# Wenri/taichi_3d_gaussian_splatting

Measured on AMD Instinct MI355X. Metric: fps fwd+bwd @1920x1080 (run as 1920x1088), 5e5 Gaussians, higher is better.
Workload: dtype f32; 1 GPU; cfg3_headline: synth(N=500000, 1920x1088, sigma0=0.02, sh_deg=3, seed 0), fwd+bwd, 1 view(s) per GPU per step, the 8 poses of BASELINE config 4 cycled (rank r, step k: pose (r + k) mod 8); points=500000, parallelism=view-parallel x1, 1 view(s) per rank per step, all-reduce per step, views_per_rank=1, poses_cycled=8, forward_sizing=predicted, rehearsal=False, backward_hook=True

## Files before the change

taichi_3d_gaussian_splatting_amd/csrc/gs_api.hip:

```cpp
#include "../../include/gs_rasterizer.h"
#include "gs_common.h"

#include <algorithm>
#include <atomic>
#include <chrono>
#include <initializer_list>
#include <mutex>
#include <string>
#include <vector>
#include <cstdio>
#include <cstring>
#include <cstdlib>

static thread_local std::string g_last_error;

static int fail(int code, const std::string& msg)
{
    g_last_error = msg;
    return code;
}

#define HIP_TRY(expr)                                                                              \
    do {                                                                                           \
        hipError_t e__ = (expr);                                                                   \
// ... 55 lines not shown
    double total_ms[KID_COUNT_] = {};
    int64_t launches[KID_COUNT_] = {};
};

int gs_prof_begin(GsProf* p, int kid, hipStream_t s)
{
    if (!p || !((p->mask >> kid) & 1ull)) return -1;
    GsProf::Rec r; r.kid = kid;
    hipEvent_t* ev[2] = { &r.a, &r.b };
    for (hipEvent_t* e : ev) {
        if (!p->spare.empty()) { *e = p->spare.back(); p->spare.pop_back(); }
        else if (hipEventCreate(e) != hipSuccess) return -1;
    }
    (void)hipEventRecord(r.a, s);
    p->recs.push_back(r);
    return (int)p->recs.size() - 1;
}

void gs_prof_end(GsProf* p, int rec, hipStream_t s)
{
    if (!p || rec < 0) return;
    (void)hipEventRecord(p->recs[rec].b, s);
}

#define GS_COUNTER_SLOTS 64
struct gs_ctx {
    int device = 0;
    GsProf prof;
    std::mutex mu;
    int64_t device_bytes = 0;
    std::vector<Frame*> frames;
    int transient = -1;
    DevBuf block_counts, block_offsets, tile_block_sums, hist, scan_tmp, counters, partial, visited, zero_row, sums, loss_ws;
    DevBuf pose_scratch;
    uint8_t visit_gen = 0;
    GsCounters* host_counters = nullptr;
    GsCounters* host_counters_dev = nullptr;
    uint64_t slots_busy = 1ull;
    int32_t ticket = 0;
    int64_t counter_wait_ns = 0;
    struct { bool valid = false; int H = 0, W = 0; uint32_t K = 0; int max_code = 0; } seen;
    DevBuf order_hint;
    int order_hint_T = 0;
    bool has_stream = false;
    hipStream_t last_stream = nullptr;
    hipEvent_t switch_event = nullptr;
};

extern "C" int gs_abi_version(void) { return GS_ABI_VERSION; }
extern "C" const char* gs_last_error(void) { return g_last_error.c_str(); }

extern "C" const char* gs_kernel_names(void)
{
    return "k_filter,k_scan_tiles_publish,k_project,k_keygen,k_sort_hist,"
           "k_sort_rowscan,k_sort_scatter,k_blend_fwd,k_blend_bwd_tile,k_bwd_points,k_sum_rows,k_tile_order,k_blend_bwd_repair";
}

extern "C" int gs_create(int32_t device, gs_ctx** out)
{
    if (!out) return fail(GS_ERR_INVALID_ARGUMENT, "gs_create: out is NULL");
    int count = 0;
    HIP_TRY(hipGetDeviceCount(&count));
    if (device < 0 || device >= count) return fail(GS_ERR_INVALID_ARGUMENT, "gs_create: no such HIP device");
    HIP_TRY(hipSetDevice(device));
    gs_ctx* c = new gs_ctx();
    c->device = device;
    hipError_t e = hipHostMalloc(reinterpret_cast<void**>(&c->host_counters), sizeof(GsCounters) * GS_COUNTER_SLOTS, hipHostMallocMapped | hipHostMallocCoherent);
    if (e != hipSuccess) { delete c; return fail(GS_ERR_HIP, std::string("hipHostMalloc: ") + hipGetErrorString(e)); }
    std::memset(c->host_counters, 0, sizeof(GsCounters) * GS_COUNTER_SLOTS);
    e = hipHostGetDevicePointer(reinterpret_cast<void**>(&c->host_counters_dev), c->host_counters, 0);
    if (e != hipSuccess) { (void)hipHostFree(c->host_counters); delete c; return fail(GS_ERR_HIP, std::string("hipHostGetDevicePointer: ") + hipGetErrorString(e)); }
    e = c->counters.ensure(sizeof(GsCounters), &c->device_bytes);
    if (e == hipSuccess) e = hipMemset(c->counters.p, 0, sizeof(GsCounters));
    if (e == hipSuccess) e = hipEventCreateWithFlags(&c->switch_event, hipEventDisableTiming);
    if (e != hipSuccess) { c->counters.release(&c->device_bytes); (void)hipHostFree(c->host_counters); delete c; return fail(GS_ERR_OUT_OF_MEMORY, "gs_create: counters"); }
    *out = c;
    return GS_OK;
}

extern "C" int gs_destroy(gs_ctx* c)
{
    if (!c) return GS_OK;
    (void)hipSetDevice(c->device);
    (void)hipDeviceSynchronize();
    for (Frame* f : c->frames) { f->bufs.release(&c->device_bytes); delete f; }
    DevBuf* all[] = { &c->block_counts, &c->block_offsets, &c->tile_block_sums, &c->hist, &c->scan_tmp,
                      &c->counters, &c->partial, &c->visited, &c->zero_row, &c->sums, &c->loss_ws, &c->order_hint, &c->pose_scratch };
    for (DevBuf* b : all) b->release(&c->device_bytes);
    for (GsProf::Rec& r : c->prof.recs) { (void)hipEventDestroy(r.a); (void)hipEventDestroy(r.b); }
    for (hipEvent_t e : c->prof.spare) (void)hipEventDestroy(e);
    if (c->switch_event) (void)hipEventDestroy(c->switch_event);
    if (c->host_counters) (void)hipHostFree(c->host_counters);
    delete c;
    return GS_OK;
}

extern "C" int gs_profile_enable(gs_ctx* c, uint64_t kernel_mask)
{
    if (!c) return fail(GS_ERR_INVALID_ARGUMENT, "gs_profile_enable: ctx is NULL");
    std::lock_guard<std::mutex> lock(c->mu);
    c->prof.mask = kernel_mask;
    return GS_OK;
}

extern "C" int gs_profile_read(gs_ctx* c, double* total_ms, int64_t* launches, int32_t n, int32_t reset)
{
    if (!c || !total_ms || !launches) return fail(GS_ERR_INVALID_ARGUMENT, "gs_profile_read: NULL argument");
    std::lock_guard<std::mutex> lock(c->mu);
    HIP_TRY(hipSetDevice(c->device));
    GsProf& p = c->prof;
    for (GsProf::Rec& r : p.recs) {
        HIP_TRY(hipEventSynchronize(r.b));
        float ms = 0.0f;
        HIP_TRY(hipEventElapsedTime(&ms, r.a, r.b));
        p.total_ms[r.kid] += ms; p.launches[r.kid] += 1;
        p.spare.push_back(r.a); p.spare.push_back(r.b);
    }
    p.recs.clear();
    for (int i = 0; i < n && i < KID_COUNT_; ++i) { total_ms[i] = p.total_ms[i]; launches[i] = p.launches[i]; }
    if (reset) for (int i = 0; i < KID_COUNT_; ++i) { p.total_ms[i] = 0.0; p.launches[i] = 0; }
// ... 247 lines not shown
        GsCounters hc;
        if ((rc = read_counters(c, s, pa.ticket, 0, &hc)) != GS_OK) return rc;
        *M_out = hc.M; *K_out = hc.K;
    }
    return GS_OK;
}

static int run_records_stage(gs_ctx* c, Frame* f, const float* records, int64_t m, const gs_config* cfg, hipStream_t s,
                             GsProjectArgs* pa_out)
{
    FrameBufs& B = f->bufs;
    const int T = f->info.n_tiles;
    const size_t Mp = (size_t)(m > 0 ? m : 1);
    const size_t nb = (size_t)((m + 255) / 256);
    const int rc = grow(c, { NEED(B.rec, 64 * Mp), NEED(B.box, 8 * Mp), NEED(B.ntiles, 4 * Mp), NEED(B.depth_codes, 4 * Mp), NEED(B.offsets, 4 * Mp),
                             NEED(B.tile_start, 4 * GS_TILE_INTS(T)), NEED(B.tile_order, 4 * GS_ORDER_INTS(T)),
                             NEED(c->tile_block_sums, 4 * (nb + 1)) });
    if (rc != GS_OK) return rc;
    if (m > 0) HIP_TRY(hipMemcpyAsync(B.rec.p, records, (size_t)m * 64, hipMemcpyDeviceToDevice, s));
    GsProjectArgs pa{};
    pa.prof = &c->prof; pa.N = m; pa.H = f->info.camera_height; pa.W = f->info.camera_width; pa.depth_scale = cfg->depth_to_sort_key_scale;
    pa.v = frame_view(*f);
    pa.tile_block_sums = c->tile_block_sums.as<uint32_t>();
    pa.counters = c->counters.as<GsCounters>();
    pa.host_mirror = c->host_counters_dev; pa.ticket = ++c->ticket;
    if (c->ticket == 0x7fffffff) c->ticket = 0;
    gs_launch_boxes_from_records(pa, (int)m, s, false);
    f->max_tiles_known = false;
    HIP_TRY(hipGetLastError());
    *pa_out = pa;
    return GS_OK;
}

static int run_raster_stage(gs_ctx* c, Frame* f, const GsProjectArgs& pa, int64_t n_rows, int M_bound, uint32_t K_bound, int depth_bits,
                            const gs_config* cfg, const gs_forward_out* out, hipStream_t s, bool publish)
{
    FrameBufs& B = f->bufs;
    const int T = f->info.n_tiles, H = f->info.camera_height, W = f->info.camera_width, tiles_x = (W + GS_TILE - 1) / GS_TILE;
    static const int seg_env = []{ const char* e = getenv("GS_BWD_SEGMENTS"); return e ? (e[0] == '0' ? 0 : 1) : -1; }();
    const bool want_cuts = seg_env >= 0 ? seg_env == 1 : (int64_t)T * waves_per_tile(T) < 6144;
    int cut_cap = 0;
    if (want_cuts && f->info.kept_for_backward && !cfg->rgb_only && K_bound > 0) {
        cut_cap = (int)std::min<uint64_t>((uint64_t)K_bound / GS_SEG + (uint64_t)T + 2, 0x7fffffffu);
        if (const int rc = grow(c, { NEED(B.cuts, (size_t)cut_cap * 256 * sizeof(float4)), NEED(B.cut_mag, (size_t)cut_cap * 256 * sizeof(float2)) }))
            return rc;
    }
    f->cut_cap = cut_cap;
    const int tile_bits = bits_for((uint32_t)(T > 1 ? T - 1 : 1));
    const int key64 = depth_bits + tile_bits > 32 ? 1 : 0;
    if (depth_bits + tile_bits > 63) return fail(GS_ERR_INVALID_ARGUMENT, "sort key needs more than 63 bits");
    const size_t Kp = K_bound > 0 ? K_bound : 1;
    const size_t key_bytes = key64 ? 8 : 4;
    const size_t hist_elems = gs_sort_hist_elems(K_bound);
    if (const int rc = grow(c, { NEED(B.keys_a, key_bytes * Kp), NEED(B.keys_b, key_bytes * Kp), NEED(B.vals_a, 4 * Kp), NEED(B.vals_b, 4 * Kp),
                                 NEED(c->hist, 4 * hist_elems), NEED(c->scan_tmp, 4 * gs_scan_tmp_elems(hist_elems)) }))
        return rc;

    GsBinArgs ba{};
    ba.prof = &c->prof;
    ba.N = n_rows; ba.M = M_bound; ba.K = K_bound; ba.counters = c->counters.as<GsCounters>();
    ba.tiles_x = tiles_x; ba.depth_scale = cfg->depth_to_sort_key_scale;
    ba.depth_bits = depth_bits; ba.key_bits = depth_bits + tile_bits;
    ba.v = frame_view(*f);
    ba.tile_block_sums = pa.tile_block_sums;
    ba.counters_rw = pa.counters; ba.host_mirror = publish ? pa.host_mirror : nullptr; ba.ticket = pa.ticket;
    ba.block_offsets = pa.block_offsets; ba.block_counts = pa.block_counts;
    ba.keys_a = B.keys_a.p; ba.keys_b = B.keys_b.p; ba.key64 = key64;
    ba.vals_a = B.vals_a.as<int32_t>(); ba.vals_b = B.vals_b.as<int32_t>();
    ba.hist = c->hist.as<uint32_t>(); ba.scan_tmp = c->scan_tmp.as<uint32_t>();
    ba.keys_sorted = &f->keys_sorted; ba.vals_sorted = &f->vals_sorted;
    gs_launch_binning(ba, s);
    HIP_TRY(hipGetLastError());

    GsBlendFwdArgs fa{};
    fa.prof = &c->prof;
    fa.H = H; fa.W = W; fa.tiles_x = tiles_x; fa.rgb_only = cfg->rgb_only;
    fa.v = frame_view(*f);
    fa.key64 = key64; fa.depth_bits = depth_bits; fa.K = K_bound; fa.counters = ba.counters;
    fa.image = out->rasterized_image; fa.depth = out->rasterized_depth; fa.acc_alpha = out->pixel_accumulated_alpha;
    fa.last = out->pixel_offset_of_last_effective_point; fa.count = out->pixel_valid_point_count;
    fa.cut_cap = cut_cap;
    static const bool use_hint = []{ const char* e = getenv("GS_FWD_ORDER_HINT"); return !(e && e[0] == '0'); }();
    fa.order_hint = (use_hint && c->order_hint_T == T && T > 0) ? c->order_hint.as<int32_t>() : nullptr;
    gs_launch_blend_fwd(fa, s);
    HIP_TRY(hipGetLastError());
    f->depth_bits = depth_bits;
    f->key64 = key64;
    f->info.sort_key_bits = depth_bits + tile_bits;
    return GS_OK;
}

static int run_forward_tail(gs_ctx* c, Frame* f, const GsProjectArgs& pa, int64_t n_rows, int M_known, const gs_config* cfg,
                            const gs_forward_out* out, hipStream_t s, int* M_out, uint32_t* K_out)
{
    static const bool predict = []{ const char* e = getenv("GS_PREDICT_SIZES"); return !(e && e[0] == '0'); }();
    const int T = f->info.n_tiles, H = f->info.camera_height, W = f->info.camera_width;
    int rc;
    f->info.sizing = GS_SIZING_EXACT;
    *M_out = 0; *K_out = 0u;
    if (n_rows == 0)
        return run_raster_stage(c, f, pa, 0, 0, 0u, 1, cfg, out, s, false);
    const int tile_bits = bits_for((uint32_t)(T > 1 ? T - 1 : 1));
    bool predicted = false;
// ... 156 lines not shown
}

extern "C" int64_t gs_frame_export_count(gs_ctx* c, const gs_frame* h, gs_export what)
{
    if (!c) return -1;
    std::lock_guard<std::mutex> lock(c->mu);
    Frame* f = resolve(c, h);
    if (f && resolve_pending(c, f) != GS_OK) return -1;
    return f ? export_count(f, what) : -1;
}

extern "C" int gs_frame_export(gs_ctx* c, const gs_frame* h, gs_export what, void* dst, gs_stream stream_)
{
    if (!c) return fail(GS_ERR_INVALID_ARGUMENT, "gs_frame_export: ctx is NULL");
    if (!dst) return fail(GS_ERR_INVALID_ARGUMENT, "gs_frame_export: dst is NULL");
    if (what < 0 || what >= GS_X_COUNT_) return fail(GS_ERR_INVALID_ARGUMENT, "gs_frame_export: unknown export id");
    std::lock_guard<std::mutex> lock(c->mu);
    Frame* f;
    int rc;
    if ((rc = lookup(c, h, "gs_frame_export", true, &f)) != GS_OK) return rc;
    if (export_count(f, what) < 0) return fail(GS_ERR_STATE, "gs_frame_export: this frame does not hold that stage");
    hipStream_t s;
    if ((rc = enter_call(c, stream_, &s)) != GS_OK) return rc;
    const GsFrameView v = frame_view(*f);
    if (what == GS_X_RECORDS) {
        if (f->info.n_points_in_camera > 0)
            HIP_TRY(hipMemcpyAsync(dst, v.PA, (size_t)f->info.n_points_in_camera * 64, hipMemcpyDeviceToDevice, s));
        return GS_OK;
    }
    GsExportArgs a{};
    a.what = (int)what; a.N = f->info.n_points; a.M = (int)f->info.n_points_in_camera; a.K = (uint32_t)f->info.n_keys;
    a.T = v.T; a.depth_bits = f->depth_bits; a.key64 = f->key64;
    a.ids = v.ids; a.PA = v.PA; a.PB = v.PB; a.PC = v.PC; a.PD = v.PD;
    a.ntiles = v.ntiles; a.offsets = v.offsets;
    a.keys_sorted = v.keys_sorted; a.vals_sorted = v.vals_sorted;
    a.tile_start = v.tile_start; a.tile_end = v.tile_end; a.mask = v.mask;
    a.dst = dst;
    gs_launch_export(a, s);
    HIP_TRY(hipGetLastError());
    return GS_OK;
}

static int waves_per_tile(int n_tiles)
{
    int G = 1;
    if (const char* e = getenv("GS_BWD_WAVES_PER_TILE")) G = atoi(e);
    else if (n_tiles < 2000) G = 4;
    else if (n_tiles < 6144) G = 2;
    if (G != 1 && G != 2 && G != 4) G = 1;
    return G;
}

static int prepare_backward_blend(gs_ctx* c, const Frame* f, const float* grad_image, const float* acc_alpha, const int32_t* last,
                                  float* mag_image, float4* sums_out, int strict, hipStream_t stream, GsBackwardArgs* a_out)
{
    const uint32_t K = (uint32_t)f->info.n_keys;
    const int G = waves_per_tile(f->info.n_tiles);
    const size_t rows = (size_t)(K > 0 ? K : 1) * (size_t)G;
    const size_t flag_bytes = (rows + 15) / 16 * 16;
    hipError_t e = c->partial.ensure(rows * 12 * sizeof(float), &c->device_bytes);
    if (e != hipSuccess) return fail(GS_ERR_OUT_OF_MEMORY, "backward: partial-sum buffer");
    const size_t Mp = (size_t)(f->info.n_points_in_camera > 0 ? f->info.n_points_in_camera : 1);
    const size_t cap_before = c->visited.cap;
    e = c->visited.ensure(flag_bytes + Mp + 16, &c->device_bytes);
    if (e != hipSuccess) return fail(GS_ERR_OUT_OF_MEMORY, "backward: visited buffer");
    if (c->visited.cap != cap_before || c->visit_gen == 255) {
        HIP_TRY(hipMemsetAsync(c->visited.p, 0, c->visited.cap, stream));
// ... 418 lines not shown
```

taichi_3d_gaussian_splatting_amd/csrc/gs_common.h:

```cpp
#pragma once
#include <hip/hip_runtime.h>
#include <stdint.h>

#define GS_TILE_SZ 16

#define gs_ballot(pred) __builtin_amdgcn_ballot_w64(pred)

#ifdef GS_STATS
extern __device__ unsigned long long gs_stats_counters[32];
extern __device__ unsigned long long gs_stats_wave_times[2 * 65536];
#endif
#if defined(GS_STATS) && GS_STATS >= 2
#define GS_STAT(i, n) do { const unsigned long long gs_stat_n = (unsigned long long)(n); if (threadIdx.x % 64 == 0) atomicAdd(&gs_stats_counters[i], gs_stat_n); } while (0)
#else
#define GS_STAT(i, n) do { } while (0)
#endif
#define GS_REC(ptr, i) (ptr)[(size_t)(i) * 4]
#define GS_BOUNDARY_TILES 3
#define GS_ALPHA_EPS 0.00392156862745098f
#define GS_ALPHA_MAX 0.99f
#define GS_T_STOP 0.0001f
#define GS_NFEAT 56
#ifndef GS_SEG
#define GS_SEG 512
// ... 238 lines not shown
    int tile_ints;
    int32_t* tile_order;
    int32_t* n_heavy;
    const void* keys_sorted; const int32_t* vals_sorted;
    float4* cuts; float2* cut_mag;
};

struct GsProjectArgs {
    GsProf* prof;
    const float* point_cloud; float* features; const int8_t* invalid; const int32_t* object_id;
    int64_t N; const float* q_pc; const float* t_pc; int n_objects; const float* Kmat;
    int H, W; float near_plane, far_plane, depth_scale;
    GsFrameView v;
    int32_t* block_counts; int32_t* block_offsets; uint32_t* tile_block_sums;
    GsCounters* counters;
    GsCounters* host_mirror; int32_t ticket;
};
void gs_launch_project(const GsProjectArgs& a, hipStream_t s, bool publish);
void gs_launch_publish(const GsProjectArgs& a, int n_blocks, hipStream_t s);
void gs_launch_boxes_from_records(const GsProjectArgs& a, int M, hipStream_t s, bool publish);

struct GsBinArgs {
    GsProf* prof;
    int64_t N; int M; uint32_t K; const GsCounters* counters; int tiles_x; float depth_scale; int depth_bits; int key_bits;
    GsFrameView v;
    const uint32_t* tile_block_sums;
    GsCounters* counters_rw; GsCounters* host_mirror; int32_t ticket;
    const int32_t *block_offsets, *block_counts;
    void *keys_a, *keys_b; int32_t *vals_a, *vals_b;
    int key64;
    uint32_t* hist;
    uint32_t* scan_tmp;
    void** keys_sorted; int32_t** vals_sorted;
};
void gs_launch_binning(const GsBinArgs& a, hipStream_t s);
size_t gs_sort_hist_elems(uint32_t K);
size_t gs_scan_tmp_elems(size_t n);

struct GsBlendFwdArgs {
    GsProf* prof;
    int H, W, tiles_x; int rgb_only;
    GsFrameView v;
    int key64, depth_bits; uint32_t K; const GsCounters* counters;
    float* image; float* depth; float* acc_alpha; int32_t* last; int32_t* count;
    int cut_cap;
    const int32_t* order_hint;
};
void gs_launch_blend_fwd(const GsBlendFwdArgs& a, hipStream_t s);

struct GsBackwardArgs {
    GsProf* prof;
    int64_t N; int M; uint32_t K; int H, W, tiles_x;
    GsFrameView v;
    int32_t* order_hint;
    const float* grad_image; const float* acc_alpha; const int32_t* last;
    const float* grad_depth; const float* depth; const float* grad_alpha; int aux;
    int G;
    int item_cap;
    int heavy_factor_x2;
    int strict;
    float* partial;
    uint8_t* visited;
    uint8_t gen;
    uint8_t* touched;
    const float4* zero_row;
    const int32_t* max_tiles_hint;
    float4* sums;
    const float* point_cloud; const float* features; const int32_t* object_id; const float* Kmat;
    int sh_band; float f_color, f_high, f_s, f_q, f_alpha;
    float* grad_pc; float* grad_feat; float* grad_uv; float* mag; float* mag_image; int32_t* n_affected;
    float* hook_gpc; float* hook_gfeat; float* hook_guv; float* hook_mag;
    int32_t* hook_ids; int32_t* hook_ntiles; float* hook_depth; float* hook_uv;
    int32_t* c_num_in_camera; int32_t* c_num_pixels; float* c_vs_grad; float* c_vs_grad_avg; float* c_pos_grad; float* c_pos_grad_norm;
};
void gs_launch_backward_blend(const GsBackwardArgs& a, hipStream_t s);
void gs_launch_backward_points(const GsBackwardArgs& a, hipStream_t s);
size_t gs_pose_scratch_size(int M, int n_objects);
void gs_launch_pose_grad(const GsBackwardArgs& a, int n_objects, void* scratch, float* grad_q, float* grad_t, hipStream_t s);

struct GsExportArgs { int what; int64_t N; int M; uint32_t K; int T; int depth_bits; int key64;
    const int32_t* ids; const float4 *PA, *PB, *PC, *PD; const int32_t* ntiles; const uint32_t* offsets;
    const void* keys_sorted; const int32_t* vals_sorted; const int32_t *tile_start, *tile_end; const int8_t* mask; void* dst; };
void gs_launch_export(const GsExportArgs& a, hipStream_t s);

struct GsLossImage { const float* p; long long sc, sy, sx; int clamp; };
size_t gs_loss_maps_size(int H, int W);
size_t gs_loss_partials_floats(int H, int W);
void gs_launch_loss_forward(const GsLossImage& X, const GsLossImage& Y, int H, int W, float lambda, float* maps, float* partials, float* terms,
                            hipStream_t s);
void gs_launch_loss_backward(const GsLossImage& X, const GsLossImage& Y, int H, int W, float lambda, const float* maps, const float* upstream,
                             const GsLossImage& G, hipStream_t s);
void gs_launch_adam(float* param, const float* grad, float* m, float* v, int64_t n, float lr, float beta1, float beta2, float eps,
                    int64_t step, hipStream_t s);
void gs_launch_reg_value(const float* feat, const int8_t* invalid, int64_t N, float* workspace, float* out, hipStream_t s);
void gs_launch_reg_grad(const float* feat, const int8_t* invalid, int64_t N, const float* value_and_count, const float* upstream,
                        float* grad, hipStream_t s);

__device__ __forceinline__ void gs_controller_add(int64_t n, int32_t npix, float mag, float g0, float g1, float g2,
                                                  int32_t* num_in_camera, int32_t* num_pixels, float* vs_grad, float* vs_grad_avg,
                                                  float* pos_grad, float* pos_grad_norm)
{
    num_in_camera[n] += 1;
    num_pixels[n] += npix;
    vs_grad[n] += mag;
    const float avg = mag / (float)npix;
    vs_grad_avg[n] += (avg != avg) ? 0.0f : avg;
    pos_grad[3 * n] += g0; pos_grad[3 * n + 1] += g1; pos_grad[3 * n + 2] += g2;
    pos_grad_norm[n] += sqrtf(g0 * g0 + g1 * g1 + g2 * g2);
}

#include "../../include/gs_rasterizer.h"
void gs_launch_density_select(const gs_scene& scene, const gs_controller_accumulators& acc, const int32_t* ids, const int32_t* npix,
                              const float* depth, const float* mag, int64_t M, int remove_floaters, const gs_density_config& cfg,
                              const gs_density_plan& plan, hipStream_t s);
// ... 6 lines not shown
```

taichi_3d_gaussian_splatting_amd/csrc/k_binning.hip:

```cpp
#include "gs_common.h"
#include <type_traits>

#ifndef SORT_ROUNDS
#define SORT_ROUNDS 16
#endif
#define SORT_TILE (256 * SORT_ROUNDS)

template <typename KeyT>
__global__ __launch_bounds__(256) void k_keygen(const int32_t* __restrict__ depth_codes, const ushort4* __restrict__ boxes,
                                                const int32_t* __restrict__ ntiles,
                                                const uint32_t* __restrict__ tile_block_sums,
                                                const int32_t* __restrict__ block_offsets, const int32_t* __restrict__ block_counts,
                                                int M, int tiles_x,
                                                float depth_scale, int depth_bits, uint32_t K_cap,
                                                uint32_t* __restrict__ offsets, KeyT* __restrict__ keys,
                                                int32_t* __restrict__ vals,
                                                GsCounters* __restrict__ counters, volatile GsCounters* host_mirror, int32_t ticket)
{
    __shared__ uint32_t ws[4];
    __shared__ uint32_t wpre[4];
    __shared__ uint32_t sExcl[256 + 1];
    __shared__ ushort4 sBox[256];
    __shared__ KeyT sCode[256];
    const int first = block_offsets ? block_offsets[blockIdx.x] : (int)blockIdx.x * 256;
    const int mine = block_offsets ? block_counts[blockIdx.x] : min(256, M - first);
    const int idx = (int)threadIdx.x < mine ? first + (int)threadIdx.x : M;
    const int lane = threadIdx.x & 63, wave = __builtin_amdgcn_readfirstlane((int)(threadIdx.x >> 6));
    const bool valid = idx < M;
    const uint32_t n = valid ? (uint32_t)ntiles[idx] : 0u;
    uint32_t incl = n;
#pragma unroll
    for (int o = 1; o < 64; o <<= 1) { uint32_t t = __shfl_up(incl, o, 64); if (lane >= o) incl += t; }
    if (lane == 63) ws[wave] = incl;
    sBox[threadIdx.x] = valid ? boxes[idx] : make_ushort4(0, 1, 0, 1);
    sCode[threadIdx.x] = valid ? (KeyT)(uint32_t)depth_codes[idx] : (KeyT)0;
    uint32_t pre = 0;
    for (int j = threadIdx.x; j < (int)blockIdx.x; j += 256) pre += tile_block_sums[j];
    pre = (uint32_t)gs_wave_sum_i((int)pre);
    if (lane == 0) wpre[wave] = pre;
    __syncthreads();
    const uint32_t block_base = wpre[0] + wpre[1] + wpre[2] + wpre[3];
    const uint32_t block_total = ws[0] + ws[1] + ws[2] + ws[3];
    if (host_mirror && blockIdx.x == gridDim.x - 1 && threadIdx.x == 0)
        gs_publish_counters(counters, block_base + block_total, host_mirror, ticket);
    uint32_t woff = 0;
    for (int w = 0; w < wave; ++w) woff += ws[w];
    const uint32_t excl = woff + incl - n;
    sExcl[threadIdx.x] = excl;
    if (threadIdx.x == 0) sExcl[256] = 0xffffffffu;
    if (valid) offsets[idx] = block_base + excl;
    __syncthreads();
    for (uint32_t e = threadIdx.x; e < block_total; e += 256u) {
        int j = 0;
#pragma unroll
        for (int step = 128; step > 0; step >>= 1) if (sExcl[j + step] <= e) j += step;
        const uint32_t t = e - sExcl[j];
        const ushort4 bx = sBox[j];
        const uint32_t dv = (uint32_t)((int)bx.w - (int)bx.z);
        uint32_t tq, tr;
        if (t < (1u << 22)) {
            tq = (uint32_t)((float)t * __builtin_amdgcn_rcpf((float)dv));
            int r = (int)t - (int)(tq * dv);
            if (r < 0) { tq -= 1u; r += (int)dv; }
            if (r >= (int)dv) { tq += 1u; r -= (int)dv; }
            tr = (uint32_t)r;
        } else { tq = t / dv; tr = t - tq * dv; }
        const KeyT tile_id = (KeyT)(((uint32_t)bx.x + tq) + ((uint32_t)bx.z + tr) * (uint32_t)tiles_x);
        const uint32_t slot = block_base + e;
        if (slot < K_cap) {
            keys[slot] = (tile_id << depth_bits) | sCode[j];
            vals[slot] = first + j;
        }
    }
    (void)depth_scale;
}

template <typename KeyT>
__global__ __launch_bounds__(256) void k_sort_hist(const KeyT* __restrict__ keys, const GsCounters* __restrict__ ctr, uint32_t n_cap, int shift,
                                                   uint32_t* __restrict__ hist, int nblocks, int tiles_per_block)
{
    __shared__ uint32_t lh[256];
    const uint32_t n = min(ctr->K, n_cap);
    lh[threadIdx.x] = 0;
    __syncthreads();
    const uint64_t begin = (uint64_t)blockIdx.x * tiles_per_block * SORT_TILE;
    uint64_t end = begin + (uint64_t)tiles_per_block * SORT_TILE;
    if (end > n) end = n;
    constexpr int V = 4;
    struct alignas(sizeof(KeyT) * V) KeyVec { KeyT k[V]; };
    const uint64_t nvec = begin < end ? (end - begin) / V : 0;
    const KeyVec* kv = reinterpret_cast<const KeyVec*>(keys + begin);
    for (uint64_t i = threadIdx.x; i < nvec; i += 256) {
        const KeyVec x = kv[i];
#pragma unroll
        for (int j = 0; j < V; ++j) atomicAdd(&lh[(uint32_t)(x.k[j] >> shift) & 255u], 1u);
    }
    for (uint64_t i = begin + nvec * V + threadIdx.x; i < end; i += 256)
        atomicAdd(&lh[(uint32_t)(keys[i] >> shift) & 255u], 1u);
    __syncthreads();
    hist[threadIdx.x * nblocks + blockIdx.x] = lh[threadIdx.x];
}

__global__ __launch_bounds__(1024) void k_sort_rowscan(const uint32_t* __restrict__ hist, uint32_t* __restrict__ totals,
                                                       uint32_t* __restrict__ offsets_out, int nblocks)
{
    __shared__ uint32_t wsum[16];
    const int d = blockIdx.x, t = threadIdx.x, lane = t & 63, wave = t >> 6;
    uint32_t carry = 0;
    const uint32_t* row = hist + (size_t)d * nblocks;
    uint32_t* orow = offsets_out + (size_t)d * nblocks;
    for (int start = 0; start < nblocks; start += 1024) {
        const int i = start + t;
        const uint32_t x = i < nblocks ? row[i] : 0u;
        uint32_t incl = x;
#pragma unroll
        for (int o = 1; o < 64; o <<= 1) { uint32_t y = __shfl_up(incl, o, 64); if (lane >= o) incl += y; }
        __syncthreads();
        if (lane == 63) wsum[wave] = incl;
        __syncthreads();
        uint32_t woff = 0;
        for (int w = 0; w < wave; ++w) woff += wsum[w];
        if (i < nblocks) orow[i] = carry + woff + incl - x;
        uint32_t tot = 0;
        for (int w = 0; w < 16; ++w) tot += wsum[w];
        carry += tot;
    }
    if (t == 0) totals[d] = carry;
}

template <typename KeyT>
__global__ __launch_bounds__(256) void k_sort_scatter(const KeyT* __restrict__ keys_in, const int32_t* __restrict__ vals_in,
                                                      KeyT* __restrict__ keys_out, int32_t* __restrict__ vals_out,
                                                      const GsCounters* __restrict__ ctr, uint32_t n_cap, int shift, const uint32_t* __restrict__ hist_scanned,
                                                      const uint32_t* __restrict__ totals, int nblocks, int tiles_per_block)
{
    const uint32_t n = min(ctr->K, n_cap);
    __shared__ uint32_t cnt[4][256];
    __shared__ uint32_t gbase[256];
    __shared__ uint32_t dstart[256];
    __shared__ uint32_t wtot[4];
    __shared__ KeyT skeys[SORT_TILE];
    __shared__ int32_t svals[SORT_TILE];
    const int t = threadIdx.x, lane = t & 63, wave = t >> 6;
    const unsigned long long lt_mask = (1ull << lane) - 1ull;
    {
        const uint32_t tot = totals[t];
        uint32_t incl = tot;
#pragma unroll
        for (int o = 1; o < 64; o <<= 1) { const uint32_t y = __shfl_up(incl, o, 64); if (lane >= o) incl += y; }
        if (lane == 63) wtot[wave] = incl;
        __syncthreads();
        uint32_t woff = 0;
        for (int w = 0; w < wave; ++w) woff += wtot[w];
        gbase[t] = (woff + incl - tot) + hist_scanned[t * nblocks + blockIdx.x];
        __syncthreads();
    }
    auto do_tile = [&](auto full_tag, const uint64_t tile_base, const uint32_t tile_n) {
        constexpr bool FULL = decltype(full_tag)::value;
        cnt[0][t] = 0; cnt[1][t] = 0; cnt[2][t] = 0; cnt[3][t] = 0;
        __syncthreads();
        KeyT k[SORT_ROUNDS];
        int32_t v[SORT_ROUNDS];
        uint32_t rank[SORT_ROUNDS];
#pragma unroll
        for (int r = 0; r < SORT_ROUNDS; ++r) {
            const uint32_t li = (uint32_t)wave * (SORT_ROUNDS * 64) + r * 64 + lane;
            const bool valid = FULL || li < tile_n;
            k[r] = valid ? keys_in[tile_base + li] : (KeyT)0;
            v[r] = valid ? vals_in[tile_base + li] : 0;
        }
#pragma unroll
        for (int r = 0; r < SORT_ROUNDS; ++r) {
            const uint32_t li = (uint32_t)wave * (SORT_ROUNDS * 64) + r * 64 + lane;
            const bool valid = FULL || li < tile_n;
            const uint32_t d = (uint32_t)(k[r] >> shift) & 255u;
            const unsigned long long vm = gs_ballot(valid);
            uint32_t slo = (uint32_t)vm, shi = (uint32_t)(vm >> 32);
#pragma unroll
            for (int bit = 0; bit < 8; ++bit) {
                const int32_t mb = (int32_t)(d << (31 - bit)) >> 31;
                const unsigned long long bal = gs_ballot(mb < 0);
                slo &= ~((uint32_t)bal ^ (uint32_t)mb);
                shi &= ~((uint32_t)(bal >> 32) ^ (uint32_t)mb);
            }
            const uint32_t in_round = (uint32_t)__popc(slo & (uint32_t)lt_mask) + (uint32_t)__popc(shi & (uint32_t)(lt_mask >> 32));
            const uint32_t before = valid ? cnt[wave][d] : 0u;
            if (valid && in_round == 0) cnt[wave][d] = before + (uint32_t)__popc(slo) + (uint32_t)__popc(shi);
            rank[r] = before + in_round;
        }
        __syncthreads();
        const uint32_t c0 = cnt[0][t], c1 = cnt[1][t], c2 = cnt[2][t], c3 = cnt[3][t];
        const uint32_t tot = c0 + c1 + c2 + c3;
        uint32_t incl = tot;
#pragma unroll
        for (int o = 1; o < 64; o <<= 1) { const uint32_t y = __shfl_up(incl, o, 64); if (lane >= o) incl += y; }
        if (lane == 63) wtot[wave] = incl;
        __syncthreads();
        uint32_t woff = 0;
        for (int w = 0; w < wave; ++w) woff += wtot[w];
        const uint32_t ds = woff + incl - tot;
        dstart[t] = ds;
        cnt[0][t] = ds; cnt[1][t] = ds + c0; cnt[2][t] = ds + c0 + c1; cnt[3][t] = ds + c0 + c1 + c2;
        __syncthreads();
#pragma unroll
        for (int r = 0; r < SORT_ROUNDS; ++r) {
            const uint32_t li = (uint32_t)wave * (SORT_ROUNDS * 64) + r * 64 + lane;
            if (FULL || li < tile_n) {
                const uint32_t d = (uint32_t)(k[r] >> shift) & 255u;
                const uint32_t ipos = cnt[wave][d] + rank[r];
                skeys[ipos] = k[r];
                svals[ipos] = v[r];
            }
        }
        __syncthreads();
#pragma unroll
        for (int r = 0; r < SORT_ROUNDS; ++r) {
            const uint32_t idx = (uint32_t)r * 256u + t;
            if (FULL || idx < tile_n) {
                const KeyT kk = skeys[idx];
                const uint32_t d = (uint32_t)(kk >> shift) & 255u;
                const uint32_t pos = gbase[d] + (idx - dstart[d]);
                keys_out[pos] = kk;
                vals_out[pos] = svals[idx];
            }
        }
        __syncthreads();
        gbase[t] += tot;
        __syncthreads();
    };
    for (int tile = 0; tile < tiles_per_block; ++tile) {
        const uint64_t tile_base = ((uint64_t)blockIdx.x * tiles_per_block + tile) * SORT_TILE;
        if (tile_base >= n) break;
        const uint32_t tile_n = (uint32_t)((n - tile_base) < SORT_TILE ? (n - tile_base) : SORT_TILE);
        if (tile_n == SORT_TILE) do_tile(std::true_type{}, tile_base, tile_n);
        else do_tile(std::false_type{}, tile_base, tile_n);
    }
}

static void sort_geometry(uint32_t K, int* nblocks, int* tiles_per_block)
{
    uint32_t tiles = (K + SORT_TILE - 1) / SORT_TILE;
    uint32_t target = tiles < 1024u ? tiles : 1024u;
    if (target == 0) target = 1;
    *tiles_per_block = (int)((tiles + target - 1) / target);
    if (*tiles_per_block < 1) *tiles_per_block = 1;
    *nblocks = (int)((tiles + *tiles_per_block - 1) / *tiles_per_block);
    if (*nblocks < 1) *nblocks = 1;
}

size_t gs_sort_hist_elems(uint32_t K)
{
    int nb, tpb;
    sort_geometry(K, &nb, &tpb);
    return (size_t)2 * 256 * nb;
}

size_t gs_scan_tmp_elems(size_t) { return 256; }

template <typename KeyT>
static void launch_binning_t(const GsBinArgs& a, hipStream_t s)
{
    KeyT* keys_a = reinterpret_cast<KeyT*>(a.keys_a);
    KeyT* keys_b = reinterpret_cast<KeyT*>(a.keys_b);
    *a.keys_sorted = a.keys_a;
    *a.vals_sorted = a.vals_a;
    if (a.N == 0 || a.M == 0) return;
    const unsigned kg_blocks = a.block_offsets ? (unsigned)((a.N + 255) / 256) : (unsigned)((a.M + 255) / 256);
    GS_TIMED(a.prof, KID_KEYGEN, s, k_keygen<KeyT><<<kg_blocks, 256, 0, s>>>(
        a.v.depth_codes, a.v.box, a.v.ntiles, a.tile_block_sums, a.block_offsets, a.block_counts, a.M, a.tiles_x, a.depth_scale, a.depth_bits, a.K, a.v.offsets, keys_a, a.vals_a,
        a.counters_rw, a.host_mirror, a.ticket));
    if (a.K == 0) return;
    int nb, tpb;
    sort_geometry(a.K, &nb, &tpb);
    KeyT *kin = keys_a, *kout = keys_b;
    int32_t *vin = a.vals_a, *vout = a.vals_b;
    for (int shift = 0; shift < a.key_bits; shift += 8) {
        uint32_t* offs = a.hist + (size_t)256 * nb;
        GS_TIMED(a.prof, KID_SORT_HIST, s, k_sort_hist<KeyT><<<nb, 256, 0, s>>>(kin, a.counters, a.K, shift, a.hist, nb, tpb));
        GS_TIMED(a.prof, KID_SORT_ROWSCAN, s, k_sort_rowscan<<<256, 1024, 0, s>>>(a.hist, a.scan_tmp, offs, nb));
        GS_TIMED(a.prof, KID_SORT_SCATTER, s, k_sort_scatter<KeyT><<<nb, 256, 0, s>>>(kin, vin, kout, vout, a.counters, a.K, shift, offs, a.scan_tmp, nb, tpb));
        KeyT* tk = kin; kin = kout; kout = tk;
        int32_t* tv = vin; vin = vout; vout = tv;
    }
    *a.keys_sorted = kin;
    *a.vals_sorted = vin;
}

void gs_launch_binning(const GsBinArgs& a, hipStream_t s)
{
    if (a.key64) launch_binning_t<uint64_t>(a, s);
    else launch_binning_t<uint32_t>(a, s);
}
```

taichi_3d_gaussian_splatting_amd/csrc/k_export.hip:

```cpp
#include "../../include/gs_rasterizer.h"
#include "gs_common.h"

__global__ void k_export(GsExportArgs a)
{
    const int64_t i = (int64_t)blockIdx.x * blockDim.x + threadIdx.x;
    switch (a.what) {
    case GS_X_POINT_ID_IN_CAMERA_LIST: if (i < a.M) ((int32_t*)a.dst)[i] = a.ids[i]; break;
    case GS_X_POINT_UV: if (i < a.M) { float4 v = GS_REC(a.PA, i); ((float*)a.dst)[2 * i] = v.x; ((float*)a.dst)[2 * i + 1] = v.y; } break;
    case GS_X_POINT_IN_CAMERA: if (i < a.M) { float4 v = GS_REC(a.PD, i); float* d = (float*)a.dst + 3 * i; d[0] = v.x; d[1] = v.y; d[2] = v.z; } break;
    case GS_X_POINT_UV_CONIC_AND_RESCALE: if (i < a.M) { float4 A = GS_REC(a.PA, i), B = GS_REC(a.PB, i); ((float4*)a.dst)[i] = make_float4(A.z, A.w, B.x, B.y); } break;
    case GS_X_POINT_ALPHA_AFTER_ACTIVATION: if (i < a.M) ((float*)a.dst)[i] = GS_REC(a.PB, i).z; break;
    case GS_X_POINT_COLOR: if (i < a.M) { float4 v = GS_REC(a.PC, i); float* d = (float*)a.dst + 3 * i; d[0] = v.x; d[1] = v.y; d[2] = v.z; } break;
    case GS_X_POINT_RADII: if (i < a.M) ((float*)a.dst)[i] = GS_REC(a.PD, i).w; break;
    case GS_X_NUM_OVERLAP_TILES: if (i < a.M) ((int32_t*)a.dst)[i] = a.ntiles[i]; break;
    case GS_X_ACCUMULATED_NUM_OVERLAP_TILES: if (i < a.M) ((int64_t*)a.dst)[i] = (int64_t)a.offsets[i]; break;
    case GS_X_SORT_KEY:
        if (i < (int64_t)a.K) {
            uint64_t k = a.key64 ? ((const uint64_t*)a.keys_sorted)[i] : (uint64_t)((const uint32_t*)a.keys_sorted)[i];
            int64_t tile = (int64_t)(k >> a.depth_bits);
            int64_t code = (int64_t)(k & ((1ull << a.depth_bits) - 1ull));
            ((int64_t*)a.dst)[i] = code + (tile << 32);
        }
        break;
    case GS_X_POINT_OFFSET_WITH_SORT_KEY: if (i < (int64_t)a.K) ((int32_t*)a.dst)[i] = a.vals_sorted[i]; break;
    case GS_X_TILE_POINTS_START: if (i < a.T) ((int32_t*)a.dst)[i] = a.tile_start[i]; break;
    case GS_X_TILE_POINTS_END: if (i < a.T) ((int32_t*)a.dst)[i] = a.tile_end[i]; break;
    case GS_X_POINT_DEPTH: if (i < a.M) ((float*)a.dst)[i] = GS_REC(a.PB, i).w; break;
    case GS_X_POINT_IN_CAMERA_MASK: if (i < a.N) ((int8_t*)a.dst)[i] = a.mask[i]; break;
    default: break;
    }
}

void gs_launch_export(const GsExportArgs& a, hipStream_t s)
{
    int64_t n = a.M;
    if (a.what == GS_X_SORT_KEY || a.what == GS_X_POINT_OFFSET_WITH_SORT_KEY) n = a.K;
    else if (a.what == GS_X_TILE_POINTS_START || a.what == GS_X_TILE_POINTS_END) n = a.T;
    else if (a.what == GS_X_POINT_IN_CAMERA_MASK) n = a.N;
    if (n <= 0) return;
    k_export<<<(unsigned)((n + 255) / 256), 256, 0, s>>>(a);
}
```

Measured before the change: 1443 frames/s.

## Pre-sort points by low depth bits to drop radix passes over tile keys

Before key generation, the visible points are radix-sorted by the low 8-bit digits of their depth code. Key generation then emits tile/depth keys in that permuted order, so the large key sort can start at a higher shift and skip one or more of its passes. This trades a full pass over K keys for passes over M points, plus a per-block tile sum over the permutation. It only kicks in when there are at least 2M pairs and at least 7 pairs per point. The accumulated-offsets export is now computed by a separate single-block scan because keygen offsets no longer match the original point order.

Measured after the change: 1462 frames/s (median of 6 runs). 1.01x the previous value.

```diff
diff --git a/taichi_3d_gaussian_splatting_amd/csrc/gs_api.hip b/taichi_3d_gaussian_splatting_amd/csrc/gs_api.hip
--- a/taichi_3d_gaussian_splatting_amd/csrc/gs_api.hip
+++ b/taichi_3d_gaussian_splatting_amd/csrc/gs_api.hip
@@ -111,6 +111,7 @@
     std::vector<Frame*> frames;
     int transient = -1;
     DevBuf block_counts, block_offsets, tile_block_sums, hist, scan_tmp, counters, partial, visited, zero_row, sums, loss_ws;
+    DevBuf pt_sort;
     DevBuf pose_scratch;
     uint8_t visit_gen = 0;
     GsCounters* host_counters = nullptr;
@@ -164,7 +165,7 @@
     (void)hipDeviceSynchronize();
     for (Frame* f : c->frames) { f->bufs.release(&c->device_bytes); delete f; }
     DevBuf* all[] = { &c->block_counts, &c->block_offsets, &c->tile_block_sums, &c->hist, &c->scan_tmp,
-                      &c->counters, &c->partial, &c->visited, &c->zero_row, &c->sums, &c->loss_ws, &c->order_hint, &c->pose_scratch };
+                      &c->counters, &c->partial, &c->visited, &c->zero_row, &c->sums, &c->loss_ws, &c->order_hint, &c->pose_scratch, &c->pt_sort };
     for (DevBuf* b : all) b->release(&c->device_bytes);
     for (GsProf::Rec& r : c->prof.recs) { (void)hipEventDestroy(r.a); (void)hipEventDestroy(r.b); }
     for (hipEvent_t e : c->prof.spare) (void)hipEventDestroy(e);
@@ -478,6 +479,21 @@
     return GS_OK;
 }
 
+#define SORT_POINT_MIN_PAIRS 2000000u
+#define SORT_POINT_MIN_PAIRS_PER_POINT 7u
+static int sort_point_passes(int depth_bits, int key_bits, int M_bound, uint32_t K_bound)
+{
+    static const int forced = []{ const char* e = getenv("GS_SORT_POINT_PASSES"); return e && e[0] >= '0' && e[0] <= '2' ? e[0] - '0' : -1; }();
+    if (M_bound <= 0) return 0;
+    const int m_max = (depth_bits + 7) / 8;
+    if (forced >= 0) return std::min(forced, m_max);
+    if (K_bound < SORT_POINT_MIN_PAIRS || (uint64_t)K_bound < (uint64_t)SORT_POINT_MIN_PAIRS_PER_POINT * (uint64_t)M_bound) return 0;
+    const int passes_now = (key_bits + 7) / 8;
+    for (int m = 1; m <= m_max; ++m)
+        if ((key_bits - std::min(8 * m, depth_bits) + 7) / 8 < passes_now) return m;
+    return 0;
+}
+
 static int run_raster_stage(gs_ctx* c, Frame* f, const GsProjectArgs& pa, int64_t n_rows, int M_bound, uint32_t K_bound, int depth_bits,
                             const gs_config* cfg, const gs_forward_out* out, hipStream_t s, bool publish)
 {
@@ -497,9 +513,12 @@
     if (depth_bits + tile_bits > 63) return fail(GS_ERR_INVALID_ARGUMENT, "sort key needs more than 63 bits");
     const size_t Kp = K_bound > 0 ? K_bound : 1;
     const size_t key_bytes = key64 ? 8 : 4;
-    const size_t hist_elems = gs_sort_hist_elems(K_bound);
+    const int point_passes = sort_point_passes(depth_bits, depth_bits + tile_bits, M_bound, K_bound);
+    const size_t Mp = ((size_t)(M_bound > 0 ? M_bound : 1) + 3) & ~(size_t)3;
+    const size_t hist_elems = std::max(gs_sort_hist_elems(K_bound), point_passes ? gs_point_sort_hist_elems((uint32_t)M_bound) : (size_t)0);
     if (const int rc = grow(c, { NEED(B.keys_a, key_bytes * Kp), NEED(B.keys_b, key_bytes * Kp), NEED(B.vals_a, 4 * Kp), NEED(B.vals_b, 4 * Kp),
-                                 NEED(c->hist, 4 * hist_elems), NEED(c->scan_tmp, 4 * gs_scan_tmp_elems(hist_elems)) }))
+                                 NEED(c->hist, 4 * hist_elems), NEED(c->scan_tmp, 4 * gs_scan_tmp_elems(hist_elems)),
+                                 NEED(c->pt_sort, point_passes ? 4 * (4 * Mp + Mp / 256 + 2) : 0) }))
         return rc;
 
     GsBinArgs ba{};
@@ -515,6 +534,13 @@
     ba.vals_a = B.vals_a.as<int32_t>(); ba.vals_b = B.vals_b.as<int32_t>();
     ba.hist = c->hist.as<uint32_t>(); ba.scan_tmp = c->scan_tmp.as<uint32_t>();
     ba.keys_sorted = &f->keys_sorted; ba.vals_sorted = &f->vals_sorted;
+    ba.point_passes = point_passes;
+    if (point_passes) {
+        uint32_t* w = c->pt_sort.as<uint32_t>();
+        ba.pt_keys[0] = w; ba.pt_keys[1] = w + Mp;
+        ba.pt_vals[0] = reinterpret_cast<int32_t*>(w + 2 * Mp); ba.pt_vals[1] = reinterpret_cast<int32_t*>(w + 3 * Mp);
+        ba.perm_block_sums = w + 4 * Mp;
+    }
     gs_launch_binning(ba, s);
     HIP_TRY(hipGetLastError());
 
@@ -737,7 +763,7 @@
     a.what = (int)what; a.N = f->info.n_points; a.M = (int)f->info.n_points_in_camera; a.K = (uint32_t)f->info.n_keys;
     a.T = v.T; a.depth_bits = f->depth_bits; a.key64 = f->key64;
     a.ids = v.ids; a.PA = v.PA; a.PB = v.PB; a.PC = v.PC; a.PD = v.PD;
-    a.ntiles = v.ntiles; a.offsets = v.offsets;
+    a.ntiles = v.ntiles;
     a.keys_sorted = v.keys_sorted; a.vals_sorted = v.vals_sorted;
     a.tile_start = v.tile_start; a.tile_end = v.tile_end; a.mask = v.mask;
     a.dst = dst;
diff --git a/taichi_3d_gaussian_splatting_amd/csrc/gs_common.h b/taichi_3d_gaussian_splatting_amd/csrc/gs_common.h
--- a/taichi_3d_gaussian_splatting_amd/csrc/gs_common.h
+++ b/taichi_3d_gaussian_splatting_amd/csrc/gs_common.h
@@ -294,9 +294,12 @@
     uint32_t* hist;
     uint32_t* scan_tmp;
     void** keys_sorted; int32_t** vals_sorted;
+    int point_passes;
+    uint32_t* pt_keys[2]; int32_t* pt_vals[2]; uint32_t* perm_block_sums;
 };
 void gs_launch_binning(const GsBinArgs& a, hipStream_t s);
 size_t gs_sort_hist_elems(uint32_t K);
+size_t gs_point_sort_hist_elems(uint32_t M);
 size_t gs_scan_tmp_elems(size_t n);
 
 struct GsBlendFwdArgs {
@@ -341,7 +344,7 @@
 void gs_launch_pose_grad(const GsBackwardArgs& a, int n_objects, void* scratch, float* grad_q, float* grad_t, hipStream_t s);
 
 struct GsExportArgs { int what; int64_t N; int M; uint32_t K; int T; int depth_bits; int key64;
-    const int32_t* ids; const float4 *PA, *PB, *PC, *PD; const int32_t* ntiles; const uint32_t* offsets;
+    const int32_t* ids; const float4 *PA, *PB, *PC, *PD; const int32_t* ntiles;
     const void* keys_sorted; const int32_t* vals_sorted; const int32_t *tile_start, *tile_end; const int8_t* mask; void* dst; };
 void gs_launch_export(const GsExportArgs& a, hipStream_t s);
 
diff --git a/taichi_3d_gaussian_splatting_amd/csrc/k_binning.hip b/taichi_3d_gaussian_splatting_amd/csrc/k_binning.hip
--- a/taichi_3d_gaussian_splatting_amd/csrc/k_binning.hip
+++ b/taichi_3d_gaussian_splatting_amd/csrc/k_binning.hip
@@ -5,8 +5,11 @@
 #define SORT_ROUNDS 16
 #endif
 #define SORT_TILE (256 * SORT_ROUNDS)
-
-template <typename KeyT>
+#ifndef POINT_SORT_ROUNDS
+#define POINT_SORT_ROUNDS 4
+#endif
+
+template <typename KeyT, bool PERM>
 __global__ __launch_bounds__(256) void k_keygen(const int32_t* __restrict__ depth_codes, const ushort4* __restrict__ boxes,
                                                 const int32_t* __restrict__ ntiles,
                                                 const uint32_t* __restrict__ tile_block_sums,
@@ -15,16 +18,27 @@
                                                 float depth_scale, int depth_bits, uint32_t K_cap,
                                                 uint32_t* __restrict__ offsets, KeyT* __restrict__ keys,
                                                 int32_t* __restrict__ vals,
-                                                GsCounters* __restrict__ counters, volatile GsCounters* host_mirror, int32_t ticket)
+                                                GsCounters* __restrict__ counters, volatile GsCounters* host_mirror, int32_t ticket,
+                                                const int32_t* __restrict__ perm, const uint32_t* __restrict__ perm_codes)
 {
     __shared__ uint32_t ws[4];
     __shared__ uint32_t wpre[4];
     __shared__ uint32_t sExcl[256 + 1];
     __shared__ ushort4 sBox[256];
     __shared__ KeyT sCode[256];
-    const int first = block_offsets ? block_offsets[blockIdx.x] : (int)blockIdx.x * 256;
-    const int mine = block_offsets ? block_counts[blockIdx.x] : min(256, M - first);
-    const int idx = (int)threadIdx.x < mine ? first + (int)threadIdx.x : M;
+    __shared__ int32_t sIdx[PERM ? 256 : 1];
+    int first, mine, idx;
+    if constexpr (PERM) {
+        const int m_real = min(counters->M, M);
+        first = (int)blockIdx.x * 256;
+        mine = min(256, m_real - first);
+        idx = (int)threadIdx.x < mine ? perm[first + (int)threadIdx.x] : M;
+        sIdx[threadIdx.x] = idx;
+    } else {
+        first = block_offsets ? block_offsets[blockIdx.x] : (int)blockIdx.x * 256;
+        mine = block_offsets ? block_counts[blockIdx.x] : min(256, M - first);
+        idx = (int)threadIdx.x < mine ? first + (int)threadIdx.x : M;
+    }
     const int lane = threadIdx.x & 63, wave = __builtin_amdgcn_readfirstlane((int)(threadIdx.x >> 6));
     const bool valid = idx < M;
     const uint32_t n = valid ? (uint32_t)ntiles[idx] : 0u;
@@ -33,7 +47,8 @@
     for (int o = 1; o < 64; o <<= 1) { uint32_t t = __shfl_up(incl, o, 64); if (lane >= o) incl += t; }
     if (lane == 63) ws[wave] = incl;
     sBox[threadIdx.x] = valid ? boxes[idx] : make_ushort4(0, 1, 0, 1);
-    sCode[threadIdx.x] = valid ? (KeyT)(uint32_t)depth_codes[idx] : (KeyT)0;
+    if constexpr (PERM) sCode[threadIdx.x] = valid ? (KeyT)perm_codes[first + (int)threadIdx.x] : (KeyT)0;
+    else sCode[threadIdx.x] = valid ? (KeyT)(uint32_t)depth_codes[idx] : (KeyT)0;
     uint32_t pre = 0;
     for (int j = threadIdx.x; j < (int)blockIdx.x; j += 256) pre += tile_block_sums[j];
     pre = (uint32_t)gs_wave_sum_i((int)pre);
@@ -69,22 +84,23 @@
         const uint32_t slot = block_base + e;
         if (slot < K_cap) {
             keys[slot] = (tile_id << depth_bits) | sCode[j];
-            vals[slot] = first + j;
+            if constexpr (PERM) vals[slot] = sIdx[j]; else vals[slot] = first + j;
         }
     }
     (void)depth_scale;
 }
 
-template <typename KeyT>
+template <typename KeyT, bool POINTS = false, int ROUNDS = SORT_ROUNDS>
 __global__ __launch_bounds__(256) void k_sort_hist(const KeyT* __restrict__ keys, const GsCounters* __restrict__ ctr, uint32_t n_cap, int shift,
                                                    uint32_t* __restrict__ hist, int nblocks, int tiles_per_block)
 {
+    constexpr uint32_t TILE = 256 * ROUNDS;
     __shared__ uint32_t lh[256];
-    const uint32_t n = min(ctr->K, n_cap);
+    const uint32_t n = min(POINTS ? (uint32_t)ctr->M : ctr->K, n_cap);
     lh[threadIdx.x] = 0;
     __syncthreads();
-    const uint64_t begin = (uint64_t)blockIdx.x * tiles_per_block * SORT_TILE;
-    uint64_t end = begin + (uint64_t)tiles_per_block * SORT_TILE;
+    const uint64_t begin = (uint64_t)blockIdx.x * tiles_per_block * TILE;
+    uint64_t end = begin + (uint64_t)tiles_per_block * TILE;
     if (end > n) end = n;
     constexpr int V = 4;
     struct alignas(sizeof(KeyT) * V) KeyVec { KeyT k[V]; };
@@ -128,19 +144,20 @@
     if (t == 0) totals[d] = carry;
 }
 
-template <typename KeyT>
+template <typename KeyT, bool POINTS = false, int ROUNDS = SORT_ROUNDS>
 __global__ __launch_bounds__(256) void k_sort_scatter(const KeyT* __restrict__ keys_in, const int32_t* __restrict__ vals_in,
                                                       KeyT* __restrict__ keys_out, int32_t* __restrict__ vals_out,
                                                       const GsCounters* __restrict__ ctr, uint32_t n_cap, int shift, const uint32_t* __restrict__ hist_scanned,
                                                       const uint32_t* __restrict__ totals, int nblocks, int tiles_per_block)
 {
-    const uint32_t n = min(ctr->K, n_cap);
+    constexpr uint32_t TILE = 256 * ROUNDS;
+    const uint32_t n = min(POINTS ? (uint32_t)ctr->M : ctr->K, n_cap);
     __shared__ uint32_t cnt[4][256];
     __shared__ uint32_t gbase[256];
     __shared__ uint32_t dstart[256];
     __shared__ uint32_t wtot[4];
-    __shared__ KeyT skeys[SORT_TILE];
-    __shared__ int32_t svals[SORT_TILE];
+    __shared__ KeyT skeys[TILE];
+    __shared__ int32_t svals[TILE];
     const int t = threadIdx.x, lane = t & 63, wave = t >> 6;
     const unsigned long long lt_mask = (1ull << lane) - 1ull;
     {
@@ -159,19 +176,20 @@
         constexpr bool FULL = decltype(full_tag)::value;
         cnt[0][t] = 0; cnt[1][t] = 0; cnt[2][t] = 0; cnt[3][t] = 0;
         __syncthreads();
-        KeyT k[SORT_ROUNDS];
-        int32_t v[SORT_ROUNDS];
-        uint32_t rank[SORT_ROUNDS];
-#pragma unroll
-        for (int r = 0; r < SORT_ROUNDS; ++r) {
-            const uint32_t li = (uint32_t)wave * (SORT_ROUNDS * 64) + r * 64 + lane;
+        KeyT k[ROUNDS];
+        int32_t v[ROUNDS];
+        uint32_t rank[ROUNDS];
+#pragma unroll
+        for (int r = 0; r < ROUNDS; ++r) {
+            const uint32_t li = (uint32_t)wave * (ROUNDS * 64) + r * 64 + lane;
             const bool valid = FULL || li < tile_n;
             k[r] = valid ? keys_in[tile_base + li] : (KeyT)0;
-            v[r] = valid ? vals_in[tile_base + li] : 0;
-        }
-#pragma unroll
-        for (int r = 0; r < SORT_ROUNDS; ++r) {
-            const uint32_t li = (uint32_t)wave * (SORT_ROUNDS * 64) + r * 64 + lane;
+            if (POINTS && vals_in == nullptr) v[r] = (int32_t)(tile_base + li);
+            else v[r] = valid ? vals_in[tile_base + li] : 0;
+        }
+#pragma unroll
+        for (int r = 0; r < ROUNDS; ++r) {
+            const uint32_t li = (uint32_t)wave * (ROUNDS * 64) + r * 64 + lane;
             const bool valid = FULL || li < tile_n;
             const uint32_t d = (uint32_t)(k[r] >> shift) & 255u;
             const unsigned long long vm = gs_ballot(valid);
@@ -203,8 +221,8 @@
         cnt[0][t] = ds; cnt[1][t] = ds + c0; cnt[2][t] = ds + c0 + c1; cnt[3][t] = ds + c0 + c1 + c2;
         __syncthreads();
 #pragma unroll
-        for (int r = 0; r < SORT_ROUNDS; ++r) {
-            const uint32_t li = (uint32_t)wave * (SORT_ROUNDS * 64) + r * 64 + lane;
+        for (int r = 0; r < ROUNDS; ++r) {
+            const uint32_t li = (uint32_t)wave * (ROUNDS * 64) + r * 64 + lane;
             if (FULL || li < tile_n) {
                 const uint32_t d = (uint32_t)(k[r] >> shift) & 255u;
                 const uint32_t ipos = cnt[wave][d] + rank[r];
@@ -214,7 +232,7 @@
         }
         __syncthreads();
 #pragma unroll
-        for (int r = 0; r < SORT_ROUNDS; ++r) {
+        for (int r = 0; r < ROUNDS; ++r) {
             const uint32_t idx = (uint32_t)r * 256u + t;
             if (FULL || idx < tile_n) {
                 const KeyT kk = skeys[idx];
@@ -229,17 +247,17 @@
         __syncthreads();
     };
     for (int tile = 0; tile < tiles_per_block; ++tile) {
-        const uint64_t tile_base = ((uint64_t)blockIdx.x * tiles_per_block + tile) * SORT_TILE;
+        const uint64_t tile_base = ((uint64_t)blockIdx.x * tiles_per_block + tile) * TILE;
         if (tile_base >= n) break;
-        const uint32_t tile_n = (uint32_t)((n - tile_base) < SORT_TILE ? (n - tile_base) : SORT_TILE);
-        if (tile_n == SORT_TILE) do_tile(std::true_type{}, tile_base, tile_n);
+        const uint32_t tile_n = (uint32_t)((n - tile_base) < TILE ? (n - tile_base) : TILE);
+        if (tile_n == TILE) do_tile(std::true_type{}, tile_base, tile_n);
         else do_tile(std::false_type{}, tile_base, tile_n);
     }
 }
 
-static void sort_geometry(uint32_t K, int* nblocks, int* tiles_per_block)
-{
-    uint32_t tiles = (K + SORT_TILE - 1) / SORT_TILE;
+static void sort_geometry(uint32_t K, int* nblocks, int* tiles_per_block, uint32_t tile = SORT_TILE)
+{
+    uint32_t tiles = (K + tile - 1) / tile;
     uint32_t target = tiles < 1024u ? tiles : 1024u;
     if (target == 0) target = 1;
     *tiles_per_block = (int)((tiles + target - 1) / target);
@@ -255,7 +273,45 @@
     return (size_t)2 * 256 * nb;
 }
 
+size_t gs_point_sort_hist_elems(uint32_t M)
+{
+    int nb, tpb;
+    sort_geometry(M, &nb, &tpb, 256 * POINT_SORT_ROUNDS);
+    return (size_t)2 * 256 * nb;
+}
+
 size_t gs_scan_tmp_elems(size_t) { return 256; }
+
+__global__ __launch_bounds__(256) void k_perm_block_sums(const int32_t* __restrict__ perm, const int32_t* __restrict__ ntiles,
+                                                         const GsCounters* __restrict__ ctr, int m_cap, uint32_t* __restrict__ sums)
+{
+    __shared__ int wsum[4];
+    const int m_real = min(ctr->M, m_cap);
+    const int i = (int)blockIdx.x * 256 + (int)threadIdx.x;
+    const int n = gs_wave_sum_i(i < m_real ? ntiles[perm[i]] : 0);
+    if ((threadIdx.x & 63) == 0) wsum[threadIdx.x >> 6] = n;
+    __syncthreads();
+    if (threadIdx.x == 0) sums[blockIdx.x] = (uint32_t)(wsum[0] + wsum[1] + wsum[2] + wsum[3]);
+}
+
+static int launch_point_passes(const GsBinArgs& a, hipStream_t s)
+{
+    int nb, tpb;
+    sort_geometry((uint32_t)a.M, &nb, &tpb, 256 * POINT_SORT_ROUNDS);
+    uint32_t* offs = a.hist + (size_t)256 * nb;
+    const uint32_t* kin = reinterpret_cast<const uint32_t*>(a.v.depth_codes);
+    const int32_t* vin = nullptr;
+    int which = 0;
+    for (int p = 0; p < a.point_passes; ++p) {
+        which = p & 1;
+        GS_TIMED(a.prof, KID_SORT_HIST, s, (k_sort_hist<uint32_t, true, POINT_SORT_ROUNDS><<<nb, 256, 0, s>>>(kin, a.counters, (uint32_t)a.M, 8 * p, a.hist, nb, tpb)));
+        GS_TIMED(a.prof, KID_SORT_ROWSCAN, s, k_sort_rowscan<<<256, 1024, 0, s>>>(a.hist, a.scan_tmp, offs, nb));
+        GS_TIMED(a.prof, KID_SORT_SCATTER, s, (k_sort_scatter<uint32_t, true, POINT_SORT_ROUNDS><<<nb, 256, 0, s>>>(kin, vin, a.pt_keys[which], a.pt_vals[which], a.counters,
+                                                                                              (uint32_t)a.M, 8 * p, offs, a.scan_tmp, nb, tpb)));
+        kin = a.pt_keys[which]; vin = a.pt_vals[which];
+    }
+    return which;
+}
 
 template <typename KeyT>
 static void launch_binning_t(const GsBinArgs& a, hipStream_t s)
@@ -265,16 +321,27 @@
     *a.keys_sorted = a.keys_a;
     *a.vals_sorted = a.vals_a;
     if (a.N == 0 || a.M == 0) return;
-    const unsigned kg_blocks = a.block_offsets ? (unsigned)((a.N + 255) / 256) : (unsigned)((a.M + 255) / 256);
-    GS_TIMED(a.prof, KID_KEYGEN, s, k_keygen<KeyT><<<kg_blocks, 256, 0, s>>>(
-        a.v.depth_codes, a.v.box, a.v.ntiles, a.tile_block_sums, a.block_offsets, a.block_counts, a.M, a.tiles_x, a.depth_scale, a.depth_bits, a.K, a.v.offsets, keys_a, a.vals_a,
-        a.counters_rw, a.host_mirror, a.ticket));
+    int first_shift = 0;
+    if (a.point_passes > 0) {
+        const int w = launch_point_passes(a, s);
+        const unsigned kg_blocks = (unsigned)((a.M + 255) / 256);
+        GS_TIMED(a.prof, KID_KEYGEN, s, k_perm_block_sums<<<kg_blocks, 256, 0, s>>>(a.pt_vals[w], a.v.ntiles, a.counters, a.M, a.perm_block_sums));
+        GS_TIMED(a.prof, KID_KEYGEN, s, (k_keygen<KeyT, true><<<kg_blocks, 256, 0, s>>>(
+            a.v.depth_codes, a.v.box, a.v.ntiles, a.perm_block_sums, nullptr, nullptr, a.M, a.tiles_x, a.depth_scale, a.depth_bits, a.K, a.v.offsets, keys_a, a.vals_a,
+            a.counters_rw, a.host_mirror, a.ticket, a.pt_vals[w], a.pt_keys[w])));
+        first_shift = a.point_passes * 8 < a.depth_bits ? a.point_passes * 8 : a.depth_bits;
+    } else {
+        const unsigned kg_blocks = a.block_offsets ? (unsigned)((a.N + 255) / 256) : (unsigned)((a.M + 255) / 256);
+        GS_TIMED(a.prof, KID_KEYGEN, s, (k_keygen<KeyT, false><<<kg_blocks, 256, 0, s>>>(
+            a.v.depth_codes, a.v.box, a.v.ntiles, a.tile_block_sums, a.block_offsets, a.block_counts, a.M, a.tiles_x, a.depth_scale, a.depth_bits, a.K, a.v.offsets, keys_a, a.vals_a,
+            a.counters_rw, a.host_mirror, a.ticket, nullptr, nullptr)));
+    }
     if (a.K == 0) return;
     int nb, tpb;
     sort_geometry(a.K, &nb, &tpb);
     KeyT *kin = keys_a, *kout = keys_b;
     int32_t *vin = a.vals_a, *vout = a.vals_b;
-    for (int shift = 0; shift < a.key_bits; shift += 8) {
+    for (int shift = first_shift; shift < a.key_bits; shift += 8) {
         uint32_t* offs = a.hist + (size_t)256 * nb;
         GS_TIMED(a.prof, KID_SORT_HIST, s, k_sort_hist<KeyT><<<nb, 256, 0, s>>>(kin, a.counters, a.K, shift, a.hist, nb, tpb));
         GS_TIMED(a.prof, KID_SORT_ROWSCAN, s, k_sort_rowscan<<<256, 1024, 0, s>>>(a.hist, a.scan_tmp, offs, nb));
diff --git a/taichi_3d_gaussian_splatting_amd/csrc/k_export.hip b/taichi_3d_gaussian_splatting_amd/csrc/k_export.hip
--- a/taichi_3d_gaussian_splatting_amd/csrc/k_export.hip
+++ b/taichi_3d_gaussian_splatting_amd/csrc/k_export.hip
@@ -13,7 +13,6 @@
     case GS_X_POINT_COLOR: if (i < a.M) { float4 v = GS_REC(a.PC, i); float* d = (float*)a.dst + 3 * i; d[0] = v.x; d[1] = v.y; d[2] = v.z; } break;
     case GS_X_POINT_RADII: if (i < a.M) ((float*)a.dst)[i] = GS_REC(a.PD, i).w; break;
     case GS_X_NUM_OVERLAP_TILES: if (i < a.M) ((int32_t*)a.dst)[i] = a.ntiles[i]; break;
-    case GS_X_ACCUMULATED_NUM_OVERLAP_TILES: if (i < a.M) ((int64_t*)a.dst)[i] = (int64_t)a.offsets[i]; break;
     case GS_X_SORT_KEY:
         if (i < (int64_t)a.K) {
             uint64_t k = a.key64 ? ((const uint64_t*)a.keys_sorted)[i] : (uint64_t)((const uint32_t*)a.keys_sorted)[i];
@@ -31,8 +30,33 @@
     }
 }
 
+__global__ __launch_bounds__(1024) void k_export_tile_scan(const int32_t* __restrict__ ntiles, int M, int64_t* __restrict__ dst)
+{
+    __shared__ int64_t wsum[16];
+    const int t = threadIdx.x, lane = t & 63, wave = t >> 6;
+    int64_t carry = 0;
+    for (int start = 0; start < M; start += 1024) {
+        const int i = start + t;
+        const int64_t x = i < M ? (int64_t)ntiles[i] : 0;
+        int64_t incl = x;
+#pragma unroll
+        for (int o = 1; o < 64; o <<= 1) { const int64_t y = __shfl_up(incl, o, 64); if (lane >= o) incl += y; }
+        __syncthreads();
+        if (lane == 63) wsum[wave] = incl;
+        __syncthreads();
+        int64_t woff = 0, tot = 0;
+        for (int w = 0; w < 16; ++w) { if (w < wave) woff += wsum[w]; tot += wsum[w]; }
+        if (i < M) dst[i] = carry + woff + incl - x;
+        carry += tot;
+    }
+}
+
 void gs_launch_export(const GsExportArgs& a, hipStream_t s)
 {
+    if (a.what == GS_X_ACCUMULATED_NUM_OVERLAP_TILES) {
+        if (a.M > 0) k_export_tile_scan<<<1, 1024, 0, s>>>(a.ntiles, a.M, (int64_t*)a.dst);
+        return;
+    }
     int64_t n = a.M;
     if (a.what == GS_X_SORT_KEY || a.what == GS_X_POINT_OFFSET_WITH_SORT_KEY) n = a.K;
     else if (a.what == GS_X_TILE_POINTS_START || a.what == GS_X_TILE_POINTS_END) n = a.T;
```
